# amoretti86/PSVO

Measured on AMD Instinct MI355X. Metric: particle-steps/sec, higher is better.
Workload: dtype f32

## Files before the change

### psvo_amd/csrc/bsim_bwd2_impl.h

```cpp
#pragma once
#define PSVO_BSIM_BWD_V2_UNIT 1
#include "bsim_bwd_impl.h"

namespace psvo {
PSVO_TIMERS_DEFINE(bsim_bwd2)

#define PSVO_GARG(args_type, field) ::psvo::as_global(PSVO_ARG(args_type, field))

__device__ __forceinline__ float swap_add32(float lo, float hi) {
    asm volatile("s_nop 1\n\tv_permlane32_swap_b32 %0, %1" : "+v"(lo), "+v"(hi));
    return lo + hi;
}
__device__ __forceinline__ float swap_add16(float lo, float hi) {
    asm volatile("s_nop 1\n\tv_permlane16_swap_b32 %0, %1" : "+v"(lo), "+v"(hi));
    return lo + hi;
}
__device__ __forceinline__ float row_sum16(float v) {
    v += dpp_mov<0x128, 0xF, 0xF, true>(v, v);
    v += dpp_mov<0x124, 0xF, 0xF, true>(v, v);
    v += dpp_mov<0x122, 0xF, 0xF, true>(v, v);
    v += dpp_mov<0x121, 0xF, 0xF, true>(v, v);
    return v;
}

__device__ __forceinline__ float rs_bit3(float lo, float hi) {
    float r;
    asm volatile("s_nop 1\n\t"
                 "v_add_f32_dpp %0, %1, %1 row_ror:8 row_mask:0xf bank_mask:0x3\n\t"
                 "v_add_f32_dpp %0, %2, %2 row_ror:8 row_mask:0xf bank_mask:0xc"
                 : "=&v"(r) : "v"(lo), "v"(hi));
    return r;
}
__device__ __forceinline__ float rs_bit2(float lo, float hi) {
    float r;
    asm volatile("s_nop 1\n\t"
                 "v_add_f32_dpp %0, %1, %1 row_shl:4 row_mask:0xf bank_mask:0x5\n\t"
                 "v_add_f32_dpp %0, %2, %2 row_shr:4 row_mask:0xf bank_mask:0xa"
                 : "=&v"(r) : "v"(lo), "v"(hi));
    return r;
}
template <int K>
__device__ __forceinline__ void row_reduce_scatter(const float (&v)[4 * K], float (&out)[K]) {
    float h[2 * K];
#pragma unroll
    for (int i = 0; i < 2 * K; ++i) h[i] = rs_bit3(v[i], v[2 * K + i]);
#pragma unroll
    for (int i = 0; i < K; ++i) out[i] = group_sum<4>(rs_bit2(h[i], h[K + i]));
}

typedef float f4v __attribute__((ext_vector_type(4)));
typedef __bf16 bf8v __attribute__((ext_vector_type(8)));

__device__ __forceinline__ void bf16_split3(float v, unsigned& h, unsigned& m, unsigned& l) {
    const unsigned hb = __float_as_uint(v) & 0xffff0000u;
    const float r = v - __uint_as_float(hb);
    const unsigned mb = __float_as_uint(r) & 0xffff0000u;
    const float r2 = r - __uint_as_float(mb);
    h = hb >> 16;
    m = mb >> 16;
    l = __float_as_uint(r2) >> 16;
}
__device__ __forceinline__ uint4 bf16x3_a(float v) {
    unsigned h, m, l;
    bf16_split3(v, h, m, l);
    return make_uint4(h | (h << 16), m | (h << 16), l | (m << 16), m | (l << 16));
}
__device__ __forceinline__ uint4 bf16x3_b(float v) {
    unsigned h, m, l;
    bf16_split3(v, h, m, l);
    return make_uint4(h | (m << 16), h | (l << 16), h | (m << 16), l | (m << 16));
}

template <int DX, int DY, int H, int M, int JM>
__global__ void __launch_bounds__(256, 2) bsim_bwd2_kernel(const BsimBwdArgs a) {
    using MQ = MlpLds<DX, H, DX, 1>;
    using MG = MlpLds<DX, H, DY, 1>;
    using AC = BAcc<DX>;
    constexpr int kN = AC::kSg + DY;
    constexpr int PS = (JM == 3) ? 20 : (DX == 4 && JM == 0) ? 5 : BTileSlot<DX>::kFloats;
    constexpr int FO = (JM == 3) ? 16 : 0;
    constexpr int NA = DX + 1;
    constexpr int PART = 2;
    constexpr int G = M * PART;
    constexpr int CPW = 64 / G;
    constexpr int CM = CPW * M;
    constexpr int NF = DX + 2;
    constexpr int UVS = (2 * DX + 3) & ~3;
    constexpr int JC = (JM == 0 && DX == 4) ? 2 : (JM || DX >= 3) ? 4 : 8;
    constexpr bool RO = (DX == 4) && (JM == 0);
    constexpr bool kSplitTile = (DX == 4) && (JM == 0);
    static_assert(CM == 32 && (M % 4) == 0, "two lanes per (chain, m): M in {4, 8, 16, 32}");
    extern __shared__ __attribute__((aligned(16))) float smem[];

    const int tid = threadIdx.x, lane = tid & 63, wave = tid >> 6;
    constexpr int NTB = 256, nwv = 4;
    const int B = a.B, T = a.T, N = a.N;
    const int NP = ((N + 127) / 128) * 128;
    const int nch = NP / (16 * JC);
    const int b = blockIdx.y, blk = blockIdx.x, nblk = gridDim.x;
    constexpr int cpb = nwv * CPW;
    const int cl = lane / G, part = (lane / M) & 1, m = lane % M;
    const bool h0 = (part == 0);
    const int n_raw = blk * cpb + wave * CPW + cl;
    const bool valid = n_raw < N;
    const int n = valid ? n_raw : N - 1;
    const bool srow = valid && h0;
    const bool lead = srow && (m == 0);
    const int j16 = lane & 15, g = lane >> 4;

    float* wf = smem;
    float* wg = wf + MQ::kSize;
    float* wqi = wg + MG::kSize;
    float* tile = wqi + MQ::kSize;
    float* jacc = tile + 2 * NP * PS;
    float* xch = jacc + nwv * NA * NP;
    float* uvx = xch + nwv * NF * CM;
    float* red = uvx + nwv * CM * UVS;
    float* const xw = xch + wave * NF * CM;
    float* const uw = uvx + wave * CM * UVS;
    float* const ja = jacc + wave * NA * NP;

    MQ::load(wf, a.f, tid, NTB);
    MG::load(wg, a.g, tid, NTB);
    MQ::load(wqi, a.q1inv, tid, NTB);

    const float kappa = sqrtf(0.5f * kLog2e);
    float isf[DX], rp[DX], isfk[DX], isg[DY];
#pragma unroll
    for (int d = 0; d < DX; ++d) {
        isf[d] = 1.f / a.sig_f[d];
        rp[d] = isf[d] * kappa;
        isfk[d] = isf[d] / kappa;
    }
    float ikap2 = 1.f / (kappa * kappa);
#pragma unroll
    for (int e = 0; e < DY; ++e) isg[e] = 1.f / a.sig_g[e];
    float pc[DX], pic[DX], pi1[DX], pi2[DX];
#pragma unroll
    for (int d = 0; d < DX; ++d) {
        pi1[d] = 1.f / a.sig_q1inv[d];
        pi2[d] = 1.f / a.sig_bq2[d];
        pic[d] = pi1[d] + pi2[d];
        pc[d] = 1.f / pic[d];
    }
    float s_init[DX], is_init[DX], i_isig[DX], im[DX], mi[DX];
#pragma unroll
    for (int d = 0; d < DX; ++d) {
        s_init[d] = a.sig_init[d];
        is_init[d] = 1.f / s_init[d];
        i_isig[d] = 1.f / a.isig[d];
        im[d] = a.imean[b * DX + d];
        mi[d] = a.minit[b * DX + d];
    }
    if constexpr (DX <= 2) {
        keep_in_vgpr(isf); keep_in_vgpr(rp); keep_in_vgpr(isfk); keep_in_vgpr(isg); keep_in_vgpr(ikap2);
        keep_in_vgpr(pc); keep_in_vgpr(pic); keep_in_vgpr(pi1); keep_in_vgpr(pi2);
    }
    const float ninf = -__builtin_huge_valf();
    const float aw = valid ? as_global(a.dscore)[(size_t)b * N + n] : 0.f;

    const unsigned NM = (unsigned)N * M;
    unsigned o_nm = 4u * ((unsigned)b * NM + n * M + m);
    unsigned o_dnm[DX], o_knm[DY], o_dn[DX];
#pragma unroll
    for (int d = 0; d < DX; ++d) {
        o_dnm[d] = 4u * (((unsigned)b * DX + d) * NM + n * M + m);
        o_dn[d] = 4u * (((unsigned)b * DX + d) * N + n);
    }
#pragma unroll
    for (int k = 0; k < DY; ++k) o_knm[k] = 4u * (((unsigned)b * DY + k) * NM + n * M + m);
    unsigned o_n = 4u * ((unsigned)b * N + n);
    unsigned o_d = 4u * ((unsigned)b * DX), o_k = 4u * ((unsigned)b * DY);
    const unsigned s_nm = 4u * B * NM, s_dnm = s_nm * DX, s_knm = s_nm * DY, s_dn = 4u * B * DX * N, s_n = 4u * B * N,
                   s_d = 4u * B * DX, s_k = 4u * B * DY;

    float st[DX + 1], st_l = 0.f;
    int st_t = 0;
    auto put_slot = [&](float* buf, int j, const float (&raw)[DX + 1], float l) {
        float F[DX];
#pragma unroll
        for (int d = 0; d < DX; ++d) F[d] = raw[d] * rp[d];
        const float W = j < N ? (raw[DX] - l) * kLog2e : ninf;
        if constexpr (JM == 3) {
            const float Wf = fmaxf(W, -1e30f);
            uint4* q = reinterpret_cast<uint4*>(buf + j * PS);
            q[0] = bf16x3_b(F[0]);
            q[1] = bf16x3_b(F[DX > 1 ? 1 : 0]);
            q[2] = bf16x3_b(Wf - (F[0] * F[0] + F[DX > 1 ? 1 : 0] * F[DX > 1 ? 1 : 0]));
            q[3] = bf16x3_b(1.f);
            *reinterpret_cast<float4*>(buf + j * PS + 16) = make_float4(F[0], F[DX > 1 ? 1 : 0], 0.f, 0.f);
        } else if constexpr (JM == 2) {
            *reinterpret_cast<float4*>(buf + j * PS) = make_float4(F[0], F[1], W - (F[0] * F[0] + F[DX > 1 ? 1 : 0] * F[DX > 1 ? 1 : 0]), 1.f);
        } else if constexpr (DX <= 3) {
            float4 v;
            v.x = F[0];
            v.y = DX > 1 ? F[DX > 1 ? 1 : 0] : 0.f;
            v.z = DX > 2 ? F[DX > 2 ? 2 : 0] : 0.f;
            v.w = W;
            *reinterpret_cast<float4*>(buf + j * PS) = v;
        } else if constexpr (kSplitTile) {
            *reinterpret_cast<float4*>(buf + 4 * j) = make_float4(F[0], F[1], F[2], F[3]);
            buf[4 * NP + j] = W;
        } else {
            *reinterpret_cast<float4*>(buf + j * PS) = make_float4(F[0], F[1], F[2], F[3]);
            *reinterpret_cast<float4*>(buf + j * PS + 4) = make_float4(W, 0.f, 0.f, 0.f);
        }
    };
    auto tile_entry = [&](const float* buf, int j, float (&F)[DX], float& W) {
        if constexpr (kSplitTile) {
            const float4 e = *reinterpret_cast<const float4*>(buf + 4 * j);
            F[0] = e.x; F[DX > 1 ? 1 : 0] = e.y; F[DX > 2 ? 2 : 0] = e.z; F[DX > 3 ? 3 : 0] = e.w;
            W = buf[4 * NP + j];
        } else {
            read_slot<DX>(buf + j * PS, F, W);
        }
    };
    static_assert(offsetof(BsimBwdArgs, logW) - offsetof(BsimBwdArgs, Fm) == 8 &&
                  offsetof(BsimBwdArgs, lse) - offsetof(BsimBwdArgs, Fm) == 16 && offsetof(BsimBwdArgs, Fm) % 32 == 0,
                  "BsimBwdArgs: forward-tile pointer block");
    auto get_slot = [&](int tt, int j, float (&raw)[DX + 1], gptr<const float> Fm, gptr<const float> logW) {
        const unsigned tb = (unsigned)tt * B + b;
        const unsigned jc = j < N ? j : N - 1;
#pragma unroll
        for (int d = 0; d < DX; ++d) raw[d] = ldf(Fm, 4u * ((tb * DX + d) * N + jc));
        raw[DX] = ldf(logW, 4u * (tb * N + jc));
    };
    float st2[DX + 1];
    const bool two_slots = (DX >= 3) && NP > NTB;
    auto stage_load = [&](int tt) {
        unsigned long long pt[4];
        arg_block<4>((unsigned)offsetof(BsimBwdArgs, Fm), pt);
        st_t = tt;
        const gptr<const float> p_Fm = as_global<const float>(pt[0]), p_logW = as_global<const float>(pt[1]);
        st_l = ldf(as_global<const float>(pt[2]), 4u * ((unsigned)tt * B + b));
        if (tid < NP) get_slot(tt, tid, st, p_Fm, p_logW);
        if (two_slots && tid + NTB < NP) get_slot(tt, tid + NTB, st2, p_Fm, p_logW);
    };
    auto stage_store = [&](float* buf) {
        if (tid < NP) put_slot(buf, tid, st, st_l);
        if (two_slots && tid + NTB < NP) put_slot(buf, tid + NTB, st2, st_l);
        for (int j = tid + (two_slots ? 2 : 1) * NTB; j < NP; j += NTB) {
            float raw[DX + 1];
            get_slot(st_t, j, raw, PSVO_GARG(BsimBwdArgs, Fm), PSVO_GARG(BsimBwdArgs, logW));
            put_slot(buf, j, raw, st_l);
        }
    };
    if (T >= 2) {
        stage_load(0);
        stage_store(tile);
    }
    __syncthreads();

    constexpr bool kAccLds = (DX >= 3);
    constexpr int kRowsA = 2 * DX + DY, kRowsB = 5 * DX, kSlotsB = 8;
    float acc[kAccLds ? 1 : kN];
    float* const accA = red + 16 + wave * (kRowsA * 32 + kRowsB * kSlotsB);
    float* const accB = accA + kRowsA * 32;
    auto acc_is_lead = [](int k) { return k < 4 * DX || (k >= 5 * DX && k < 6 * DX); };
    auto acc_row = [](int k) {
        return k < 4 * DX ? k : k < 5 * DX ? k - 4 * DX : k < 6 * DX ? 4 * DX + (k - 5 * DX)
               : k < 7 * DX ? DX + (k - 6 * DX) : 2 * DX + (k - 7 * DX);
    };
    const int s32 = cl * M + m;
    if constexpr (kAccLds) {
        for (int i = lane; i < kRowsA * 32 + kRowsB * kSlotsB; i += 64) accA[i] = 0.f;
    } else {
#pragma unroll
        for (int i = 0; i < kN; ++i) acc[i] = 0.f;
    }
    auto acc_add = [&](int k, float v) {
        if constexpr (kAccLds) {
            if (acc_is_lead(k)) atomicAdd(&accB[acc_row(k) * kSlotsB + cl], v);
            else atomicAdd(&accA[acc_row(k) * 32 + s32], v);
        } else {
            acc[k] += v;
        }
    };
    float dX[DX];
#pragma unroll
    for (int d = 0; d < DX; ++d) dX[d] = 0.f;

    struct StepIn {
        float eps[DX], bm[DX], xp[DX], mu1[DX], y[DY], om, lam2;
        int sel;
    };
    static_assert(offsetof(BsimBwdArgs, dscore) - offsetof(BsimBwdArgs, obs) == 56 && offsetof(BsimBwdArgs, obs) % 64 == 0 &&
                  offsetof(BsimBwdArgs, eps_b) - offsetof(BsimBwdArgs, obs) == 8 &&
                  offsetof(BsimBwdArgs, bwX) - offsetof(BsimBwdArgs, obs) == 16 &&
                  offsetof(BsimBwdArgs, sel) - offsetof(BsimBwdArgs, obs) == 24 &&
                  offsetof(BsimBwdArgs, lam2_all) - offsetof(BsimBwdArgs, obs) == 32 &&
                  offsetof(BsimBwdArgs, om_all) - offsetof(BsimBwdArgs, obs) == 40 &&
                  offsetof(BsimBwdArgs, mu1_all) - offsetof(BsimBwdArgs, obs) == 48, "BsimBwdArgs: input pointer block");
    auto load_step = [&](bool lst, bool fst, StepIn& s) {
        unsigned long long pb[8];
        arg_block<8>((unsigned)offsetof(BsimBwdArgs, obs), pb);
        const gptr<const float> p_obs = as_global<const float>(pb[0]);
        const gptr<const float> p_eps = as_global<const float>(pb[1]);
        const gptr<const float> p_bwX = as_global<const float>(pb[2]);
        const gptr<const int32_t> p_sel = as_global<const int32_t>(pb[3]);
        const gptr<const float> p_lam2 = as_global<const float>(pb[4]);
        const gptr<const float> p_om = as_global<const float>(pb[5]);
        const gptr<const float> p_mu1 = as_global<const float>(pb[6]);
        const gptr<const float> p_bm = PSVO_GARG(BsimBwdArgs, bmu2);
        s.sel = ldi(p_sel, o_n);
#pragma unroll
        for (int d = 0; d < DX; ++d) {
            s.eps[d] = ldf(p_eps, o_dnm[d]);
            s.bm[d] = ldf(p_bm, o_d + 4u * d);
            s.xp[d] = lst ? 0.f : ldf(p_bwX, o_dn[d] + s_dn);
            s.mu1[d] = lst ? 0.f : ldf(p_mu1, o_dn[d]);
        }
#pragma unroll
        for (int k = 0; k < DY; ++k) s.y[k] = ldf(p_obs, o_k + 4u * k);
        s.om = ldf(p_om, o_nm);
        s.lam2 = fst ? 0.f : ldf(p_lam2, o_nm);
    };
    auto advance = [&]() {
        o_nm += s_nm; o_n += s_n; o_d += s_d; o_k += s_k;
#pragma unroll
        for (int d = 0; d < DX; ++d) { o_dnm[d] += s_dnm; o_dn[d] += s_dn; }
#pragma unroll
        for (int k = 0; k < DY; ++k) o_knm[k] += s_knm;
    };
    auto settle = [&](StepIn& s) {
        keep_in_vgpr(s.eps); keep_in_vgpr(s.bm); keep_in_vgpr(s.xp); keep_in_vgpr(s.mu1); keep_in_vgpr(s.y);
        keep_in_vgpr(s.om); keep_in_vgpr(s.lam2);
        asm volatile("" : "+v"(s.sel));
    };
    StepIn cur_in;
    load_step(T == 1, true, cur_in);
    settle(cur_in);

    phase_skew(a.skew);
    SEC_INIT(bsim_bwd2)
    for (int t = 0; t < T; ++t) {
        SEC(0);
        const bool first = (t == 0), last = (t == T - 1);
        const float* cur = tile + ((t + 1) & 1) * NP * PS;
        float* nxt = tile + (t & 1) * NP * PS;
        constexpr bool kLateTile = (DX == 4);
        if (!kLateTile && t + 1 < T && t >= 1) stage_load(t);
        advance();
        constexpr bool kLatePrefetch = (DX >= 3);
        StepIn nxt_in;
        auto prefetch = [&]() {
            if (t + 1 < T) load_step(t + 2 == T, false, nxt_in);
            else nxt_in = StepIn{};
        };
        if (!kLatePrefetch) prefetch();
        SEC(1);

        float xp[DX], eps[DX], bm[DX], mu1[DX], mu[DX], x[DX], y[DY];
        const int sel = cur_in.sel;
#pragma unroll
        for (int d = 0; d < DX; ++d) {
            eps[d] = cur_in.eps[d];
            bm[d] = cur_in.bm[d];
            xp[d] = cur_in.xp[d];
            mu1[d] = cur_in.mu1[d];
            if (!last) {
                mu[d] = pc[d] * fmaf(pi1[d], mu1[d], pi2[d] * bm[d]);
                x[d] = fmaf(pc[d], eps[d], mu[d]);
            } else {
                mu[d] = mi[d];
                x[d] = fmaf(s_init[d], eps[d], mu[d]);
            }
        }
#pragma unroll
        for (int k = 0; k < DY; ++k) y[k] = cur_in.y[k];
        const float pi_m = valid ? exp2_fast(cur_in.om * kLog2e) : 0.f;
        const float issel = (m == sel) ? 1.f : 0.f;
        const float dphi = aw * pi_m;
        const float dlam = -aw * (issel - pi_m);

        float dxt[DX];
#pragma unroll
        for (int d = 0; d < DX; ++d) dxt[d] = h0 ? issel * dX[d] : 0.f;

        SEC(2);
        if (!first) {
            if (h0) {
#pragma unroll
                for (int d = 0; d < DX; ++d) xw[d * CM + cl * M + m] = x[d] * rp[d];
                xw[DX * CM + cl * M + m] = cur_in.lam2;
                xw[(DX + 1) * CM + cl * M + m] = dlam;
            }
            __builtin_amdgcn_fence(__ATOMIC_RELEASE, "wavefront");
            __builtin_amdgcn_wave_barrier();
            __builtin_amdgcn_fence(__ATOMIC_ACQUIRE, "wavefront");

            if constexpr (RO) {
#pragma unroll 1
                for (int r = 0; r < 2; ++r) {
                    const int it4 = 4 * (4 * r + g);
                    f2 xa[DX], xb[DX], Ua[DX], Ub[DX], Va[DX], Vb[DX];
#pragma unroll
                    for (int d = 0; d < DX; ++d) {
                        const float4 v = *reinterpret_cast<const float4*>(xw + d * CM + it4);
                        xa[d] = f2{v.x, v.y};
                        xb[d] = f2{v.z, v.w};
                        Ua[d] = Ub[d] = Va[d] = Vb[d] = f2{0.f, 0.f};
                    }
                    const float4 lq = *reinterpret_cast<const float4*>(xw + DX * CM + it4);
                    const float4 dl = *reinterpret_cast<const float4*>(xw + (DX + 1) * CM + it4);
                    const f2 lqa = f2{lq.x, lq.y}, lqb = f2{lq.z, lq.w};
                    const f2 dla = f2{dl.x, dl.y}, dlb = f2{dl.z, dl.w};
#pragma unroll 1
                    for (int c = 0; c < nch; ++c) {
                        float A2[JC][NA];
#pragma unroll
                        for (int jt = 0; jt < JC; ++jt) {
                            float F[DX], W;
                            tile_entry(cur, (c * JC + jt) * 16 + j16, F, W);
                            f2 ua[DX], ub[DX], la = f2{W, W}, lb = la;
#pragma unroll
                            for (int d = 0; d < DX; ++d) {
                                const f2 Fd = f2{F[d], F[d]};
                                ua[d] = xa[d] - Fd;
                                ub[d] = xb[d] - Fd;
                                la = pk_fma(-ua[d], ua[d], la);
                                lb = pk_fma(-ub[d], ub[d], lb);
                            }
// ... 208 lines not shown
                    if (g == 0 || DX > 3) {
#pragma unroll
                        for (int jt = 0; jt < JC; ++jt) {
                            float F[DX], W;
                            read_slot<DX>(cbase + jt * 16 * PS, F, W);
                            (void)W;
                            const int j = (c * JC + jt) * 16 + j16;
                            if constexpr (DX <= 3) {
                                const float sc = D4[jt][DX];
#pragma unroll
                                for (int d = 0; d < DX; ++d) ja[d * NP + j] = D4[jt][d] - F[d] * sc;
                                ja[DX * NP + j] = sc;
                            } else {
                                const float sc = __shfl(D4[jt][0], 16 + j16);
                                if (g == 0) {
#pragma unroll
                                    for (int d = 0; d < DX; ++d) ja[d * NP + j] = D4[jt][d] - F[d] * sc;
                                    ja[DX * NP + j] = sc;
                                }
                            }
                        }
                    }
                }
            }
#pragma unroll
            for (int r = 0; r < 2; ++r) {
                float vv[4 * 2 * DX], o[UVS];
#pragma unroll
                for (int d = 0; d < DX; ++d) {
                    vv[0 * 2 * DX + d] = Ua[r][d].x; vv[1 * 2 * DX + d] = Ua[r][d].y;
                    vv[2 * 2 * DX + d] = Ub[r][d].x; vv[3 * 2 * DX + d] = Ub[r][d].y;
                    vv[0 * 2 * DX + DX + d] = Va[r][d].x; vv[1 * 2 * DX + DX + d] = Va[r][d].y;
                    vv[2 * 2 * DX + DX + d] = Vb[r][d].x; vv[3 * 2 * DX + DX + d] = Vb[r][d].y;
                }
                float red2[2 * DX];
                row_reduce_scatter<2 * DX>(vv, red2);
#pragma unroll
                for (int e = 0; e < UVS; ++e) o[e] = e < 2 * DX ? red2[e < 2 * DX ? e : 0] : 0.f;
                if ((j16 & 3) == 0) {
                    float* dst = uw + (4 * (4 * r + g) + (j16 >> 2)) * UVS;
#pragma unroll
                    for (int e = 0; e < UVS; e += 4)
                        *reinterpret_cast<float4*>(dst + e) = make_float4(o[e], o[e + 1], o[e + 2], o[e + 3]);
                }
            }
            }
            __builtin_amdgcn_fence(__ATOMIC_RELEASE, "wavefront");
            __builtin_amdgcn_wave_barrier();
            __builtin_amdgcn_fence(__ATOMIC_ACQUIRE, "wavefront");
            SEC(3);
            if (h0) {
                float uv[UVS];
#pragma unroll
                for (int e = 0; e < UVS; e += 4) {
                    const float4 q4 = *reinterpret_cast<const float4*>(uw + (cl * M + m) * UVS + e);
                    uv[e] = q4.x; uv[e + 1] = q4.y; uv[e + 2] = q4.z; uv[e + 3] = q4.w;
                }
                if constexpr (JM >= 2) {
#pragma unroll
                    for (int d = 0; d < DX; ++d) {
                        const float xs = x[d] * rp[d], r1 = uv[d], r2 = uv[DX + d];
                        uv[d] = xs - r1;
                        uv[DX + d] = fmaf(xs, xs - 2.f * r1, r2);
                    }
                }
#pragma unroll
                for (int d = 0; d < DX; ++d) {
                    dxt[d] -= dlam * uv[d] * isfk[d];
                    acc_add(AC::kSf + d, dlam * (uv[DX + d] * ikap2 - 1.f) * isf[d]);
                }
            }
        } else {
#pragma unroll
            for (int d = 0; d < DX; ++d) {
                const float z = (x[d] - im[d]) * i_isig[d];
                const float tz = dphi * z * i_isig[d];
                if (h0) {
                    dxt[d] -= tz;
                    acc_add(AC::kSiota + d, dphi * (z * z - 1.f) * i_isig[d]);
                }
            }
        }

        if (kLatePrefetch) prefetch();
        if (kLateTile && t + 1 < T && t >= 1) stage_load(t);
        SEC(4);
        float dxp_part[DX];
#pragma unroll
        for (int d = 0; d < DX; ++d) dxp_part[d] = 0.f;
        {
            float dFo[DX];
#pragma unroll
            for (int d = 0; d < DX; ++d) dFo[d] = 0.f;
            if (!last) {
                float fmx[DX];
                MQ::template eval_part<PART>(wf, part, x, fmx);
#pragma unroll
                for (int d = 0; d < DX; ++d) fmx[d] += xor_lane<M>(fmx[d]);
#pragma unroll
                for (int d = 0; d < DX; ++d) {
                    const float z = (xp[d] - fmx[d]) * isf[d];
                    dFo[d] = dphi * z * isf[d];
                    if (h0) {
                        dxp_part[d] = -dFo[d];
                        acc_add(AC::kSf + d, dphi * (z * z - 1.f) * isf[d]);
                    }
                }
                MQ::template bwd_input_part<PART>(wf, part, x, dFo, dxt);
            }
            static_assert(offsetof(BsimBwdArgs, dFt) - offsetof(BsimBwdArgs, xt) == 8 &&
                          offsetof(BsimBwdArgs, dGt) - offsetof(BsimBwdArgs, xt) == 16 &&
                          offsetof(BsimBwdArgs, dmu1) - offsetof(BsimBwdArgs, xt) == 24 && offsetof(BsimBwdArgs, xt) % 32 == 0,
                          "BsimBwdArgs: row pointer block");
            unsigned long long pr[4];
            arg_block<4>((unsigned)offsetof(BsimBwdArgs, xt), pr);
            if (srow) {
#pragma unroll
                for (int d = 0; d < DX; ++d) {
                    stf(as_global<float>(pr[1]), o_dnm[d] - s_dnm, dFo[d]);
                    stf(as_global<float>(pr[0]), o_dnm[d] - s_dnm, x[d]);
                }
            }
            float gm[DY], dGo[DY];
            MG::template eval_part<PART>(wg, part, x, gm);
#pragma unroll
            for (int k = 0; k < DY; ++k) gm[k] += xor_lane<M>(gm[k]);
#pragma unroll
            for (int k = 0; k < DY; ++k) {
                float dmean = 1.f;
                if (a.emission) { dmean = emis_dmean(gm[k]); gm[k] = emis_mean(gm[k]); }
                const float z = (y[k] - gm[k]) * isg[k];
                dGo[k] = dphi * z * isg[k] * dmean;
                if (h0) acc_add(AC::kSg + k, dphi * (z * z - 1.f) * isg[k]);
                if (srow) stf(as_global<float>(pr[2]), o_knm[k] - s_knm, dGo[k]);
            }
            MG::template bwd_input_part<PART>(wg, part, x, dGo, dxt);
        }

        SEC(5);
        float dmu[DX], sce[DX], dxp[DX], dim[DX];
#pragma unroll
        for (int d = 0; d < DX; ++d) {
            const float v3 = (first && h0) ? dphi * (x[d] - im[d]) * i_isig[d] * i_isig[d] : 0.f;
            dmu[d] = group_sum<G>(dxt[d]);
            sce[d] = group_sum<G>(dxt[d] * eps[d]);
            dxp[d] = group_sum<G>(dxp_part[d]);
            dim[d] = first ? group_sum<G>(v3) : 0.f;
        }
        float outv[DX];
        if (!last) {
            float dmu1[DX];
#pragma unroll
            for (int d = 0; d < DX; ++d) {
                dmu1[d] = dmu[d] * pc[d] * pi1[d];
                outv[d] = dmu[d] * pc[d] * pi2[d];
                if (lead) {
                    stf(PSVO_GARG(BsimBwdArgs, dmu1), o_dn[d] - s_dn, dmu1[d]);
                    acc_add(AC::kSc + d, sce[d] + aw * pic[d]);
                    acc_add(AC::kSmm1 + d, dmu[d] * mu1[d]);
                    acc_add(AC::kSmb + d, dmu[d] * bm[d]);
                    acc_add(AC::kSmm + d, dmu[d] * mu[d]);
                }
            }
            {
                constexpr int kQS = (H / 4 < G) ? H / 4 : G;
                float dq[DX];
#pragma unroll
                for (int d = 0; d < DX; ++d) dq[d] = 0.f;
                MQ::template bwd_input_part<kQS>(wqi, (lane % G) & (kQS - 1), xp, dmu1, dq);
#pragma unroll
                for (int d = 0; d < DX; ++d) dxp[d] += group_sum<kQS>(dq[d]);
            }
        } else {
#pragma unroll
            for (int d = 0; d < DX; ++d) {
                outv[d] = dmu[d];
                if (lead) {
                    stf(PSVO_GARG(BsimBwdArgs, dmu1), o_dn[d] - s_dn, 0.f);
                    acc_add(AC::kSinit + d, sce[d] + aw * is_init[d]);
                }
            }
        }
#pragma unroll
        for (int d = 0; d < DX; ++d) dX[d] = dxp[d];
        if (lead) {
#pragma unroll
            for (int d = 0; d < DX; ++d) {
                stf(PSVO_GARG(BsimBwdArgs, dbmu2_rows), o_dn[d] - s_dn, last ? 0.f : outv[d]);
                if (last) PSVO_GARG(BsimBwdArgs, dminit_rows)[((size_t)b * DX + d) * N + n] = outv[d];
                if (first) PSVO_GARG(BsimBwdArgs, dimean_rows)[((size_t)b * DX + d) * N + n] = dim[d];
            }
        }
        SEC(6);
        __syncthreads();
        settle(nxt_in);
        cur_in = nxt_in;
        const size_t tb = (size_t)t * B + b;
        if (!first) {
            const size_t tbm = tb - B;
            const gptr<float> pF = PSVO_GARG(BsimBwdArgs, dFm_part) + (tbm * nblk + blk) * DX * N;
            const gptr<float> pW = PSVO_GARG(BsimBwdArgs, dlogW_part) + (tbm * nblk + blk) * N;
            for (int j = tid; j < N; j += NTB) {
#pragma unroll
                for (int d = 0; d < NA; ++d) {
                    const float* col = jacc + d * NP + j;
                    const float a0 = col[0], a1 = col[NA * NP], a2 = col[2 * NA * NP], a3 = col[3 * NA * NP];
                    const float s = (a0 + a1) + (a2 + a3);
                    if (d < DX) pF[d * N + j] = s * isfk[d < DX ? d : 0];
                    else pW[j] = s;
                }
            }
        }
        if (last) {
            const gptr<float> pF = PSVO_GARG(BsimBwdArgs, dFm_part) + (tb * nblk + blk) * DX * N;
            const gptr<float> pW = PSVO_GARG(BsimBwdArgs, dlogW_part) + (tb * nblk + blk) * N;
            for (int j = tid; j < N; j += NTB) {
#pragma unroll
                for (int d = 0; d < DX; ++d) pF[d * N + j] = 0.f;
                pW[j] = 0.f;
            }
        }
        SEC(7);
        if (t + 1 < T && t >= 1) stage_store(nxt);
        __syncthreads();
        SEC(8);
    }

    for (int i = 0; i < kN; ++i) {
        float v = 0.f;
        if constexpr (kAccLds) {
            if (acc_is_lead(i)) v = lane < kSlotsB ? accB[acc_row(i) * kSlotsB + lane] : 0.f;
            else v = lane < 32 ? accA[acc_row(i) * 32 + lane] : 0.f;
        } else {
#pragma unroll
            for (int k = 0; k < kN; ++k) v = (k == i) ? acc[k] : v;
        }
        v = wave_sum(v);
        if (lane == 0) red[wave] = v;
        __syncthreads();
        if (tid == 0) {
            float s = 0.f;
            for (int w = 0; w < nwv; ++w) s += red[w];
            as_global(a.sacc_part)[((size_t)b * nblk + blk) * kN + i] = s;
        }
        __syncthreads();
    }
}

static inline void bsim2_geometry(int N, int M, int& cpb, int& nblk) {
    cpb = 4 * (64 / (2 * M));
    nblk = (N + cpb - 1) / cpb;
}

static inline bool bsim2_supported(int B, int T, int N, int M, int Dx, int Dy) {
    if (pick_m(M, [](auto) { return PSVO_OK; }) != PSVO_OK) return false;
    const long long big = (long long)T * B * (Dx > Dy ? Dx : Dy) * N * M * 4;
    return big < (1ll << 32);
}

template <int DX, int DY, int H, int M>
static int launch_bsim_bwd2(const BsimBwdArgs& a, const BsimBwdOut& o, int jm, hipStream_t stream) {
    using MQ = MlpLds<DX, H, DX, 1>;
    using MG = MlpLds<DX, H, DY, 1>;
    const int PS = (jm == 3 && DX == 2) ? 20 : (DX == 4) ? 5 : BTileSlot<DX>::kFloats;
    constexpr int UVS = (2 * DX + 3) & ~3;
    int cpb, nblk;
    bsim2_geometry(a.N, M, cpb, nblk);
    const int NP = ((a.N + 127) / 128) * 128;
    const size_t lds = sizeof(float) * (2 * MQ::kSize + MG::kSize + 2 * (size_t)NP * PS + 4 * (size_t)(DX + 1) * NP +
                                        4 * (DX + 2) * 32 + 4 * 32 * UVS + 16 +
                                        (DX >= 3 ? 4 * ((2 * DX + DY) * 32 + 5 * DX * 8) : 0));
    if (lds > 160 * 1024) return PSVO_ERR_UNSUPPORTED;
    BsimBwdArgs as = a;
    as.skew = (int)(2560.0 * NP / 128.0 * (3 * DX + 4) / 10.0 * g_tune_skew_pct / 100.0);
    clear_hip_error();
    if (jm == 3 && DX == 2) {
        if constexpr (DX == 2)
            hipLaunchKernelGGL((bsim_bwd2_kernel<DX, DY, H, M, 3>), dim3(nblk, a.B), dim3(256), lds, stream, as);
    } else if (jm == 2 && DX == 2) {
        if constexpr (DX == 2)
            hipLaunchKernelGGL((bsim_bwd2_kernel<DX, DY, H, M, 2>), dim3(nblk, a.B), dim3(256), lds, stream, as);
    } else if (jm == 1 && DX == 2) {
        if constexpr (DX == 2)
            hipLaunchKernelGGL((bsim_bwd2_kernel<DX, DY, H, M, 1>), dim3(nblk, a.B), dim3(256), lds, stream, as);
    } else {
        hipLaunchKernelGGL((bsim_bwd2_kernel<DX, DY, H, M, 0>), dim3(nblk, a.B), dim3(256), lds, stream, as);
    }
    (void)o;
    return launch_status();
}

template <int DX>
int bb2_dispatch_dy(const BsimBwdArgs& a, const BsimBwdOut& o, int Dy, int H, int M, int jm, hipStream_t s) {
    return dispatch_dy_h_m(Dy, H, M, [&](auto dy, auto h, auto m) __attribute__((visibility("hidden"))) {
        return launch_bsim_bwd2<DX, dy(), h(), m()>(a, o, jm, s); });
}

}
```

### psvo_amd/csrc/filter_fwd.hip

```cpp
#include "common.h"

namespace psvo {
inline namespace PSVO_LNS {
PSVO_TIMERS_DEFINE(filter_fwd)


struct FilterArgs {
    int B, T, N;
    int resample, two_q, bootstrap, emission;
    psvo_mlp q1, f, g;
    const float *sig_q1, *sig_q2, *sig_f, *sig_g;
    const float *mu2, *m0, *sig0, *fm0, *fsig0, *obs, *eps, *u;
    const int32_t* idx_in;
    float *X, *Xanc, *Fm, *P1, *logW;
    int32_t* idx_out;
    float* lse;
};

template <int DX, int DY, int H, int MAXT, int EM = 2>
__global__ void __launch_bounds__(MAXT) filter_fwd_kernel(const FilterArgs a) {
    using MQ = MlpLds<DX, H, DX, PSVO_L>;
    using MG = MlpLds<DX, H, DY, PSVO_L>;
    extern __shared__ __attribute__((aligned(16))) float smem[];

// ... 144 lines not shown
        } else {
            total = lane_bcast(sc, 63);
        }
        const float lse_t = fmaf(kLn2, log2_fast(total), mx);
        if (tid == 0) a.lse[tb] = lse_t;

        SEC(5);
        if (a.resample) {
            cdf[tid] = sc;
#pragma unroll
            for (int d = 0; d < DX; ++d) {
                sx[d * NT + tid] = x[d];
                sp[d * NT + tid] = p1[d];
                if (!a.bootstrap) sf[d * NT + tid] = fm[d];
            }
            __syncthreads();
            SEC(6);
            int idx;
            if (a.idx_in) {
                idx = idx_c;
            } else {
                const float target = u_c * total;
                int pos = 0;
                for (int s = 1 << (31 - __clz(N)); s > 0; s >>= 1) {
                    const int p = pos + s;
                    if (p <= N && cdf[p - 1] <= target) pos = p;
                }
                idx = min(pos, N - 1);
            }
#pragma unroll
            for (int d = 0; d < DX; ++d) {
                x[d] = sx[d * NT + idx];
                mean1[d] = sp[d * NT + idx];
                fmean[d] = a.bootstrap ? mean1[d] : sf[d * NT + idx];
            }
            if (valid) {
                a.idx_out[tb * N + n] = idx;
#pragma unroll
                for (int d = 0; d < DX; ++d) a.Xanc[(tb * DX + d) * N + n] = x[d];
            }
            lnw = neg_logN;
            SEC(7);
            __syncthreads();
        } else {
#pragma unroll
            for (int d = 0; d < DX; ++d) {
                mean1[d] = p1[d];
                fmean[d] = fm[d];
            }
            if (valid) {
                a.idx_out[tb * N + n] = n;
#pragma unroll
                for (int d = 0; d < DX; ++d) a.Xanc[(tb * DX + d) * N + n] = x[d];
            }
            lnw = lw - lse_t;
            if (nw > 1) __syncthreads();
        }

#pragma unroll
        for (int d = 0; d < DX; ++d) {
            eps_c[d] = eps_n[d];
            mu2_c[d] = mu2_n[d];
        }
#pragma unroll
        for (int k = 0; k < DY; ++k) obs_c[k] = obs_n[k];
        u_c = u_n;
        idx_c = idx_n;
    }
}

template <int DX, int DY, int H, int MAXT>
__global__ void __launch_bounds__(MAXT) filter_fwd_lpp_kernel(const FilterArgs a) {
    using MQ = MlpLds<DX, H, DX, PSVO_L>;
    using MG = MlpLds<DX, H, DY, PSVO_L>;
    constexpr int P = 4;
    constexpr bool kOpaque = false;
    extern __shared__ __attribute__((aligned(16))) float smem[];

    const int tid = threadIdx.x, lane = tid & 63, wave = tid >> 6;
    const int NT = blockDim.x, nw = NT >> 6;
    const int NPT = NT / P;
    const int b = blockIdx.x, B = a.B, T = a.T, N = a.N;
    const int pn = tid >> 2, p = tid & 3;
    const int uwave = __builtin_amdgcn_readfirstlane(wave);
    const bool valid = pn < N;
    const int n = valid ? pn : N - 1;

    float* wq1 = smem;
    float* wf = wq1 + MQ::kSize;
    float* wg = wf + MQ::kSize;
    float* cdf = wg + MG::kSize;
    float* piv = cdf + NPT;
    float* sx = piv + 16;
    float* sp = sx + DX * NPT;
    float* sf = sp + DX * NPT;
    float* red = sf + DX * NPT;

    MQ::load(wq1, a.q1, tid, NT);
    if (!a.bootstrap) MQ::load(wf, a.f, tid, NT);
    MG::load(wg, a.g, tid, NT);
    const float* wfm = a.bootstrap ? wq1 : wf;
    if (tid < 16) piv[tid] = __builtin_huge_valf();

    float sq1[DX], sq2[DX], sfv[DX], s0[DX], fs0[DX], isg[DY];
    float lg = -DY * kHalfLog2Pi;
#pragma unroll
    for (int d = 0; d < DX; ++d) {
        sq1[d] = a.sig_q1[d];
        sq2[d] = a.two_q ? a.sig_q2[d] : 1.f;
        sfv[d] = a.bootstrap ? a.sig_q1[d] : a.sig_f[d];
        s0[d] = a.sig0[d];
        fs0[d] = a.fsig0[d];
    }
#pragma unroll
    for (int e = 0; e < DY; ++e) {
        const float s = a.sig_g[e];
        isg[e] = 1.f / s;
        lg -= logf(s);
    }
    const StepK<DX> K0 = make_stepk<DX>(s0, sq2, fs0, a.two_q != 0);
    const StepK<DX> K1 = make_stepk<DX>(sq1, sq2, sfv, a.two_q != 0);
    const float neg_logN = -logf((float)N);
    const float ninf = -__builtin_huge_valf();

    float mean1[DX], fmean[DX];
#pragma unroll
    for (int d = 0; d < DX; ++d) {
        mean1[d] = a.m0[b * DX + d];
        fmean[d] = a.fm0[b * DX + d];
    }
    float lnw = neg_logN;

    constexpr int kFU = DX, kFM2 = DX + 1, kFY = 2 * DX + 1, kFields = 2 * DX + 1 + DY, kSlots = (kFields + 3) / 4;
    const in_word_t* in_ptr[kSlots];
    int in_str[kSlots];
    auto field_ptr = [&](int f, const in_word_t*& q, int& st) {
        q = a.eps + (size_t)b * DX * N + n;
        st = 0;
        if (f < kFU) {
            q = a.eps + ((size_t)b * DX + f) * N + n;
            st = B * DX * N;
        } else if (f == kFU) {
            if (a.resample) {
                q = (a.idx_in ? reinterpret_cast<const in_word_t*>(a.idx_in) : static_cast<const in_word_t*>(a.u)) + (size_t)b * N + n;
                st = B * N;
            }
        } else if (f < kFY) {
            if (a.two_q) {
                q = a.mu2 + (size_t)b * DX + (f - kFM2);
                st = B * DX;
            }
        } else if (f < kFields) {
            q = a.obs + (size_t)b * DY + (f - kFY);
            st = B * DY;
        }
    };
#pragma unroll
    for (int s = 0; s < kSlots; ++s) {
        field_ptr(4 * s, in_ptr[s], in_str[s]);
#pragma unroll
        for (int j = 1; j < 4; ++j) {
            const in_word_t* q;
            int st;
            field_ptr(4 * s + j, q, st);
            in_ptr[s] = (p == j) ? q : in_ptr[s];
            in_str[s] = (p == j) ? st : in_str[s];
        }
    }
    float eps_c[DX], mu2_c[DX], obs_c[DY], u_c = 0.f;
    int idx_c = 0;
    float raw_n[kSlots];
    auto issue_inputs = [&]() {
#pragma unroll
        for (int s = 0; s < kSlots; ++s) {
            raw_n[s] = *in_ptr[s];
            in_ptr[s] += in_str[s];
        }
    };
    auto take_inputs = [&]() {
#pragma unroll
        for (int d = 0; d < DX; ++d) {
            eps_c[d] = quad_field(raw_n, d);
            const float m = quad_field(raw_n, kFM2 + d);
            mu2_c[d] = a.two_q ? m : 0.f;
        }
#pragma unroll
        for (int k = 0; k < DY; ++k) obs_c[k] = quad_field(raw_n, kFY + k);
        u_c = quad_field(raw_n, kFU);
        idx_c = __builtin_bit_cast(int, u_c);
    };
    issue_inputs();
    take_inputs();
    __syncthreads();

    SEC_INIT(filter_fwd)
    auto step = [&](auto first_tag, const int t) {
        SEC(0);
        const size_t tb = (size_t)t * B + b;
        const StepK<DX> K = decltype(first_tag)::value ? K0 : K1;
        if (t + 1 < T) issue_inputs();

        SEC(1);
        float mu[DX], x[DX];
#pragma unroll
        for (int d = 0; d < DX; ++d) {
            mu[d] = a.two_q ? K.c[d] * fmaf(K.i1[d], mean1[d], K.i2[d] * mu2_c[d]) : mean1[d];
            x[d] = fmaf(K.c[d], eps_c[d], mu[d]);
        }
        const float q_lp = diag_lp<DX>(x, mu, K.ic, K.lq);
        const float f_lp = diag_lp<DX>(x, fmean, K.ifs, K.lf);

        SEC(2);
        int zo = 0;
        if (kOpaque) asm volatile("" : "+v"(zo));
        float gm[DY], p1[DX], fm[DX];
        MG::template eval_part<P>(wg + zo, p, x, gm);
        MQ::template eval_part<P>(wq1 + zo, p, x, p1);
        if (!a.bootstrap) MQ::template eval_part<P>(wfm + zo, p, x, fm);
#pragma unroll
        for (int k = 0; k < DY; ++k) gm[k] = group_sum<P>(gm[k]);
        if (a.emission) {
#pragma unroll
            for (int k = 0; k < DY; ++k) gm[k] = emis_mean(gm[k]);
        }
#pragma unroll
        for (int d = 0; d < DX; ++d) {
            p1[d] = group_sum<P>(p1[d]);
            fm[d] = a.bootstrap ? p1[d] : group_sum<P>(fm[d]);
        }
        const float g_lp = diag_lp<DY>(obs_c, gm, isg, lg);
        float lw = f_lp + g_lp - q_lp + lnw;
        if (!valid) lw = ninf;

        if (valid) {
            if (p == 0) {
#pragma unroll
                for (int d = 0; d < DX; ++d) a.X[(tb * DX + d) * N + n] = x[d];
                a.logW[tb * N + n] = lw;
            } else if (p == 1) {
#pragma unroll
                for (int d = 0; d < DX; ++d) a.Fm[(tb * DX + d) * N + n] = fm[d];
            } else if (p == 2 && a.P1) {
#pragma unroll
                for (int d = 0; d < DX; ++d) a.P1[(tb * DX + d) * N + n] = p1[d];
            }
        }

        SEC(3);
        const float wmx = wave_max(lw);
        const float wbase = (wmx == ninf) ? 0.f : wmx;
        const float w = (valid && p == 0) ? exp2_fast((lw - wbase) * kLog2e) : 0.f;
        float sc = wave_incl_scan(w, lane);
        if (lane == 63) {
            red[wave] = wmx;
            red[16 + wave] = sc;
        }
        if (a.resample) {
            if (p == 1) {
#pragma unroll
                for (int d = 0; d < DX; ++d) sx[d * NPT + pn] = x[d];
            } else if (p == 2) {
#pragma unroll
                for (int d = 0; d < DX; ++d) sp[d * NPT + pn] = p1[d];
            } else if (p == 3 && !a.bootstrap) {
#pragma unroll
                for (int d = 0; d < DX; ++d) sf[d * NPT + pn] = fm[d];
            }
        }
        SEC(4);
        __syncthreads();
        SEC(5);
        const int li = lane & 15;
        const float m_i = li < nw ? red[li] : ninf;
        const float s_i = li < nw ? red[16 + li] : 0.f;
        const float gmx = lane_bcast(group_max<16>(m_i), 0);
        const float gbase = (gmx == ninf) ? 0.f : gmx;
        const float v_i = s_i * exp2_fast((m_i - gbase) * kLog2e);
        const float pre = group_incl_scan<16>(v_i, li);
        const float total = lane_bcast(pre, nw - 1);
        const float off = uwave > 0 ? lane_bcast(pre, max(uwave - 1, 0)) : 0.f;
        sc = fmaf(sc, exp2_fast((wbase - gbase) * kLog2e), off);
        const float lse_t = fmaf(kLn2, log2_fast(total), gmx);
        if (tid == 3) a.lse[tb] = lse_t;

        SEC(6);
        if (a.resample) {
            if (p == 0) {
                cdf[pn] = sc;
                if ((pn & 15) == 15) piv[pn >> 4] = sc;
            }
            __syncthreads();
            SEC(7);
            int idx;
            if (a.idx_in) {
                idx = idx_c;
            } else {
                const float target = u_c * total;
                const float4 pv = *reinterpret_cast<const float4*>(piv + 4 * p);
                float c1 = (pv.x <= target ? 1.f : 0.f) + (pv.y <= target ? 1.f : 0.f) +
                           (pv.z <= target ? 1.f : 0.f) + (pv.w <= target ? 1.f : 0.f);
                c1 = group_sum<P>(c1);
                const int blk = min((int)c1, (NPT >> 4) - 1);
                const float4 cv = *reinterpret_cast<const float4*>(cdf + 16 * blk + 4 * p);
                float c2 = (cv.x <= target ? 1.f : 0.f) + (cv.y <= target ? 1.f : 0.f) +
                           (cv.z <= target ? 1.f : 0.f) + (cv.w <= target ? 1.f : 0.f);
                c2 = group_sum<P>(c2);
                idx = min(16 * blk + (int)c2, N - 1);
            }
#pragma unroll
            for (int d = 0; d < DX; ++d) {
                x[d] = sx[d * NPT + idx];
                mean1[d] = sp[d * NPT + idx];
                fmean[d] = a.bootstrap ? mean1[d] : sf[d * NPT + idx];
            }
            if (valid) {
                if (p == 3) a.idx_out[tb * N + n] = idx;
                if (p == 0) {
#pragma unroll
                    for (int d = 0; d < DX; ++d) a.Xanc[(tb * DX + d) * N + n] = x[d];
                }
            }
            lnw = neg_logN;
            SEC(8);
            __syncthreads();
            SEC(9);
        } else {
#pragma unroll
            for (int d = 0; d < DX; ++d) {
                mean1[d] = p1[d];
                fmean[d] = fm[d];
            }
            if (valid) {
                if (p == 3) a.idx_out[tb * N + n] = n;
                if (p == 0) {
#pragma unroll
                    for (int d = 0; d < DX; ++d) a.Xanc[(tb * DX + d) * N + n] = x[d];
                }
            }
            lnw = lw - lse_t;
            __syncthreads();
        }

        take_inputs();
    };
    step(std::true_type{}, 0);
    for (int t = 1; t < T; ++t) step(std::false_type{}, t);
}

template <int DX, int DY, int H>
static int launch_filter(const FilterArgs& a, hipStream_t stream) {
    using MQ = MlpLds<DX, H, DX, PSVO_L>;
    using MG = MlpLds<DX, H, DY, PSVO_L>;
    constexpr bool kLppOk = (H % 16 == 0) && (PSVO_L == 2 || (H <= 32 && DX <= 3) || H == 16);
    if constexpr (kLppOk) {
        if (a.N <= 128) {
            const int NT4 = (4 * a.N + 63) & ~63;
            const int NPT = NT4 / 4;
            const size_t lds4 = sizeof(float) * (2 * MQ::kSize + MG::kSize + NPT + 16 + 3 * DX * NPT + 32);
            clear_hip_error();
            hipLaunchKernelGGL((filter_fwd_lpp_kernel<DX, DY, H, 512>), dim3(a.B), dim3(NT4), lds4, stream, a);
            return launch_status();
        }
    }
    const int NT = (a.N + 63) & ~63;
    const size_t lds = sizeof(float) * (2 * MQ::kSize + MG::kSize + NT + 3 * DX * NT + 48);
    clear_hip_error();
    if (NT <= 256 && a.emission)
        hipLaunchKernelGGL((filter_fwd_kernel<DX, DY, H, 256, 1>), dim3(a.B), dim3(NT), lds, stream, a);
    else if (NT <= 256)
        hipLaunchKernelGGL((filter_fwd_kernel<DX, DY, H, 256, 0>), dim3(a.B), dim3(NT), lds, stream, a);
    else
        hipLaunchKernelGGL((filter_fwd_kernel<DX, DY, H, 512>), dim3(a.B), dim3(NT), lds, stream, a);
    return launch_status();
}

}
}

PSVO_L2_DECL(psvo_filter_forward)
PSVO_ENTRY(psvo_filter_forward)(const psvo_desc* desc, const psvo_mlp* q1, const psvo_mlp* f, const psvo_mlp* g,
                                   const float* sig_q1, const float* sig_q2, const float* sig_f,
                                   const float* sig_g, const float* mu2, const float* m0, const float* sig0,
                                   const float* fm0, const float* fsig0, const float* obs, const float* eps,
                                   const float* u, const int32_t* idx_in, float* X, float* Xanc, float* Fm, float* P1,
                                   float* logW, int32_t* idx_out, float* lse, void* stream) {
    using namespace psvo;
    if (!desc_layers_ok(desc) || !desc_emission_ok(desc)) return PSVO_ERR_UNSUPPORTED;
#if PSVO_L == 1
    if (desc && desc->layers == 2)
        return psvo_filter_forward_l2(desc, q1, f, g, sig_q1, sig_q2, sig_f, sig_g, mu2, m0, sig0, fm0, fsig0, obs,
            eps, u, idx_in, X, Xanc, Fm, P1, logW, idx_out, lse, stream);
#endif
    if (!mlp_layers_ok(q1) || !mlp_layers_ok(f) || !mlp_layers_ok(g)) return PSVO_ERR_INVALID;
    if (!desc || !q1 || !g || !sig_q1 || !sig_g || !m0 || !sig0 || !fm0 || !fsig0 || !obs || !eps || !X ||
        !Xanc || !Fm || !logW || !idx_out || !lse)
        return PSVO_ERR_INVALID;
    if (desc->B <= 0 || desc->T <= 0 || desc->N <= 0) return PSVO_ERR_INVALID;
    if (desc->two_q && (!mu2 || !sig_q2)) return PSVO_ERR_INVALID;
    if (!desc->bootstrap && (!f || !sig_f)) return PSVO_ERR_INVALID;
    if (desc->resample && !u && !idx_in) return PSVO_ERR_INVALID;
    if (desc->N > 512) return PSVO_ERR_UNSUPPORTED;

    FilterArgs a;
    a.B = desc->B; a.T = desc->T; a.N = desc->N;
    a.resample = desc->resample; a.two_q = desc->two_q; a.bootstrap = desc->bootstrap; a.emission = desc->emission;
    a.q1 = *q1; a.f = desc->bootstrap ? *q1 : *f; a.g = *g;
    a.sig_q1 = sig_q1; a.sig_q2 = sig_q2; a.sig_f = sig_f; a.sig_g = sig_g;
    a.mu2 = mu2; a.m0 = m0; a.sig0 = sig0; a.fm0 = fm0; a.fsig0 = fsig0;
    a.obs = obs; a.eps = eps; a.u = u; a.idx_in = idx_in;
    a.X = X; a.Xanc = Xanc; a.Fm = Fm; a.P1 = P1; a.logW = logW; a.idx_out = idx_out; a.lse = lse;
    hipStream_t s = static_cast<hipStream_t>(stream);
    return dispatch_shape(desc->Dx, desc->Dy, desc->H, [&](auto dx, auto dy, auto h) {
        return launch_filter<dx(), dy(), h()>(a, s); });
}
```

Before: 258.6 million.

## Double-buffer LDS staging to drop per-step barriers in bwd and filter kernels

In the backward simulation kernel, the Jacobian accumulator is double-buffered when LDS allows (DX<=3), so the tile stage-store moves before the existing barrier and the second per-step barrier is removed. In the lpp filter kernel, the per-step staging area (cdf, particle state, reductions) is double-buffered by timestep parity. The resampling pivot search now computes block pivots from the scan partial sums in registers instead of writing rescaled CDF and pivots to LDS, which removes two barriers per step. The cost is more LDS, which can lower occupancy, plus more register work to rescale CDF entries during the search.

```diff
diff --git a/psvo_amd/csrc/bsim_bwd2_impl.h b/psvo_amd/csrc/bsim_bwd2_impl.h
--- a/psvo_amd/csrc/bsim_bwd2_impl.h
+++ b/psvo_amd/csrc/bsim_bwd2_impl.h
@@ -69,6 +69,17 @@
     unsigned h, m, l;
     bf16_split3(v, h, m, l);
     return make_uint4(h | (m << 16), h | (l << 16), h | (m << 16), l | (m << 16));
+}
+
+template <int DX, int DY, int H>
+__host__ __device__ constexpr int bsim2_lds_floats(int NP, int PS, int njb) {
+    constexpr int UVS = (2 * DX + 3) & ~3;
+    return 2 * MlpLds<DX, H, DX, 1>::kSize + MlpLds<DX, H, DY, 1>::kSize + 2 * NP * PS + njb * 4 * (DX + 1) * NP +
+           4 * (DX + 2) * 32 + 4 * 32 * UVS + 16 + (DX >= 3 ? 4 * ((2 * DX + DY) * 32 + 5 * DX * 8) : 0);
+}
+template <int DX, int DY, int H>
+__host__ __device__ constexpr int bsim2_jacc_copies(int NP, int PS) {
+    return (DX <= 3 && 4 * bsim2_lds_floats<DX, DY, H>(NP, PS, 2) <= 80 * 1024) ? 2 : 1;
 }
 
 template <int DX, int DY, int H, int M, int JM>
@@ -89,6 +100,7 @@
     constexpr int JC = (JM == 0 && DX == 4) ? 2 : (JM || DX >= 3) ? 4 : 8;
     constexpr bool RO = (DX == 4) && (JM == 0);
     constexpr bool kSplitTile = (DX == 4) && (JM == 0);
+    constexpr bool kOneBarrier = (DX <= 3);
     static_assert(CM == 32 && (M % 4) == 0, "two lanes per (chain, m): M in {4, 8, 16, 32}");
     extern __shared__ __attribute__((aligned(16))) float smem[];
 
@@ -112,13 +124,14 @@
     float* wg = wf + MQ::kSize;
     float* wqi = wg + MG::kSize;
     float* tile = wqi + MQ::kSize;
+    const int njb = kOneBarrier ? bsim2_jacc_copies<DX, DY, H>(NP, PS) : 1;
+    const bool one_barrier = kOneBarrier && njb == 2;
     float* jacc = tile + 2 * NP * PS;
-    float* xch = jacc + nwv * NA * NP;
+    float* xch = jacc + njb * nwv * NA * NP;
     float* uvx = xch + nwv * NF * CM;
     float* red = uvx + nwv * CM * UVS;
     float* const xw = xch + wave * NF * CM;
     float* const uw = uvx + wave * CM * UVS;
-    float* const ja = jacc + wave * NA * NP;
 
     MQ::load(wf, a.f, tid, NTB);
     MG::load(wg, a.g, tid, NTB);
@@ -174,7 +187,7 @@
     const unsigned s_nm = 4u * B * NM, s_dnm = s_nm * DX, s_knm = s_nm * DY, s_dn = 4u * B * DX * N, s_n = 4u * B * N,
                    s_d = 4u * B * DX, s_k = 4u * B * DY;
 
-    float st[DX + 1], st_l = 0.f;
+    float st[DX + 1] = {}, st_l = 0.f;
     int st_t = 0;
     auto put_slot = [&](float* buf, int j, const float (&raw)[DX + 1], float l) {
         float F[DX];
@@ -225,7 +238,7 @@
         for (int d = 0; d < DX; ++d) raw[d] = ldf(Fm, 4u * ((tb * DX + d) * N + jc));
         raw[DX] = ldf(logW, 4u * (tb * N + jc));
     };
-    float st2[DX + 1];
+    float st2[DX + 1] = {};
     const bool two_slots = (DX >= 3) && NP > NTB;
     auto stage_load = [&](int tt) {
         unsigned long long pt[4];
@@ -338,6 +351,8 @@
         const bool first = (t == 0), last = (t == T - 1);
         const float* cur = tile + ((t + 1) & 1) * NP * PS;
         float* nxt = tile + (t & 1) * NP * PS;
+        float* const jacc_t = jacc + (t & (njb - 1)) * nwv * NA * NP;
+        float* const ja = jacc_t + wave * NA * NP;
         constexpr bool kLateTile = (DX == 4);
         if (!kLateTile && t + 1 < T && t >= 1) stage_load(t);
         advance();
@@ -712,6 +727,11 @@
             }
         }
 
+        if constexpr (kOneBarrier) {
+            keep_in_vgpr(st);
+            keep_in_vgpr(st_l);
+            if constexpr (DX >= 3) keep_in_vgpr(st2);
+        }
         if (kLatePrefetch) prefetch();
         if (kLateTile && t + 1 < T && t >= 1) stage_load(t);
         SEC(4);
@@ -822,6 +842,7 @@
             }
         }
         SEC(6);
+        if (one_barrier && t + 1 < T && t >= 1) stage_store(nxt);
         __syncthreads();
         settle(nxt_in);
         cur_in = nxt_in;
@@ -833,7 +854,7 @@
             for (int j = tid; j < N; j += NTB) {
 #pragma unroll
                 for (int d = 0; d < NA; ++d) {
-                    const float* col = jacc + d * NP + j;
+                    const float* col = jacc_t + d * NP + j;
                     const float a0 = col[0], a1 = col[NA * NP], a2 = col[2 * NA * NP], a3 = col[3 * NA * NP];
                     const float s = (a0 + a1) + (a2 + a3);
                     if (d < DX) pF[d * N + j] = s * isfk[d < DX ? d : 0];
@@ -851,8 +872,10 @@
             }
         }
         SEC(7);
-        if (t + 1 < T && t >= 1) stage_store(nxt);
-        __syncthreads();
+        if (!one_barrier) {
+            if (t + 1 < T && t >= 1) stage_store(nxt);
+            __syncthreads();
+        }
         SEC(8);
     }
 
@@ -890,16 +913,11 @@
 
 template <int DX, int DY, int H, int M>
 static int launch_bsim_bwd2(const BsimBwdArgs& a, const BsimBwdOut& o, int jm, hipStream_t stream) {
-    using MQ = MlpLds<DX, H, DX, 1>;
-    using MG = MlpLds<DX, H, DY, 1>;
     const int PS = (jm == 3 && DX == 2) ? 20 : (DX == 4) ? 5 : BTileSlot<DX>::kFloats;
-    constexpr int UVS = (2 * DX + 3) & ~3;
     int cpb, nblk;
     bsim2_geometry(a.N, M, cpb, nblk);
     const int NP = ((a.N + 127) / 128) * 128;
-    const size_t lds = sizeof(float) * (2 * MQ::kSize + MG::kSize + 2 * (size_t)NP * PS + 4 * (size_t)(DX + 1) * NP +
-                                        4 * (DX + 2) * 32 + 4 * 32 * UVS + 16 +
-                                        (DX >= 3 ? 4 * ((2 * DX + DY) * 32 + 5 * DX * 8) : 0));
+    const size_t lds = sizeof(float) * (size_t)bsim2_lds_floats<DX, DY, H>(NP, PS, bsim2_jacc_copies<DX, DY, H>(NP, PS));
     if (lds > 160 * 1024) return PSVO_ERR_UNSUPPORTED;
     BsimBwdArgs as = a;
     as.skew = (int)(2560.0 * NP / 128.0 * (3 * DX + 4) / 10.0 * g_tune_skew_pct / 100.0);
diff --git a/psvo_amd/csrc/filter_fwd.hip b/psvo_amd/csrc/filter_fwd.hip
--- a/psvo_amd/csrc/filter_fwd.hip
+++ b/psvo_amd/csrc/filter_fwd.hip
@@ -250,25 +250,19 @@
     const int NPT = NT / P;
     const int b = blockIdx.x, B = a.B, T = a.T, N = a.N;
     const int pn = tid >> 2, p = tid & 3;
-    const int uwave = __builtin_amdgcn_readfirstlane(wave);
     const bool valid = pn < N;
     const int n = valid ? pn : N - 1;
 
     float* wq1 = smem;
     float* wf = wq1 + MQ::kSize;
     float* wg = wf + MQ::kSize;
-    float* cdf = wg + MG::kSize;
-    float* piv = cdf + NPT;
-    float* sx = piv + 16;
-    float* sp = sx + DX * NPT;
-    float* sf = sp + DX * NPT;
-    float* red = sf + DX * NPT;
+    const int blk_floats = (1 + 3 * DX) * NPT + 32;
+    float* const stage = wg + MG::kSize;
 
     MQ::load(wq1, a.q1, tid, NT);
     if (!a.bootstrap) MQ::load(wf, a.f, tid, NT);
     MG::load(wg, a.g, tid, NT);
     const float* wfm = a.bootstrap ? wq1 : wf;
-    if (tid < 16) piv[tid] = __builtin_huge_valf();
 
     float sq1[DX], sq2[DX], sfv[DX], s0[DX], fs0[DX], isg[DY];
     float lg = -DY * kHalfLog2Pi;
@@ -366,6 +360,11 @@
         SEC(0);
         const size_t tb = (size_t)t * B + b;
         const StepK<DX> K = decltype(first_tag)::value ? K0 : K1;
+        float* const cdf = stage + (t & 1) * blk_floats;
+        float* const sx = cdf + NPT;
+        float* const sp = sx + DX * NPT;
+        float* const sf = sp + DX * NPT;
+        float* const red = sf + DX * NPT;
         if (t + 1 < T) issue_inputs();
 
         SEC(1);
@@ -418,13 +417,15 @@
         const float wmx = wave_max(lw);
         const float wbase = (wmx == ninf) ? 0.f : wmx;
         const float w = (valid && p == 0) ? exp2_fast((lw - wbase) * kLog2e) : 0.f;
-        float sc = wave_incl_scan(w, lane);
+        const float sc = wave_incl_scan(w, lane);
         if (lane == 63) {
             red[wave] = wmx;
             red[16 + wave] = sc;
         }
         if (a.resample) {
-            if (p == 1) {
+            if (p == 0) {
+                cdf[pn] = sc;
+            } else if (p == 1) {
 #pragma unroll
                 for (int d = 0; d < DX; ++d) sx[d * NPT + pn] = x[d];
             } else if (p == 2) {
@@ -446,32 +447,28 @@
         const float v_i = s_i * exp2_fast((m_i - gbase) * kLog2e);
         const float pre = group_incl_scan<16>(v_i, li);
         const float total = lane_bcast(pre, nw - 1);
-        const float off = uwave > 0 ? lane_bcast(pre, max(uwave - 1, 0)) : 0.f;
-        sc = fmaf(sc, exp2_fast((wbase - gbase) * kLog2e), off);
         const float lse_t = fmaf(kLn2, log2_fast(total), gmx);
         if (tid == 3) a.lse[tb] = lse_t;
 
         SEC(6);
         if (a.resample) {
-            if (p == 0) {
-                cdf[pn] = sc;
-                if ((pn & 15) == 15) piv[pn >> 4] = sc;
-            }
-            __syncthreads();
-            SEC(7);
             int idx;
             if (a.idx_in) {
                 idx = idx_c;
             } else {
                 const float target = u_c * total;
-                const float4 pv = *reinterpret_cast<const float4*>(piv + 4 * p);
-                float c1 = (pv.x <= target ? 1.f : 0.f) + (pv.y <= target ? 1.f : 0.f) +
-                           (pv.z <= target ? 1.f : 0.f) + (pv.w <= target ? 1.f : 0.f);
-                c1 = group_sum<P>(c1);
-                const int blk = min((int)c1, (NPT >> 4) - 1);
+                const float base_i = (m_i == ninf) ? 0.f : m_i;
+                const float E_i = exp2_fast((base_i - gbase) * kLog2e);
+                const float off_i = dpp_mov<0x111, 0xF, 0xF, true>(0.f, pre);
+                const float piv_i = li < nw ? fmaf(s_i, E_i, off_i) : __builtin_huge_valf();
+                int c1 = 0;
+#pragma unroll
+                for (int i = 0; i < MAXT / 64; ++i) c1 += (lane_bcast(piv_i, i) <= target) ? 1 : 0;
+                const int blk = min(c1, nw - 1);
+                const float E_b = lane_fetch(E_i, blk), off_b = lane_fetch(off_i, blk);
                 const float4 cv = *reinterpret_cast<const float4*>(cdf + 16 * blk + 4 * p);
-                float c2 = (cv.x <= target ? 1.f : 0.f) + (cv.y <= target ? 1.f : 0.f) +
-                           (cv.z <= target ? 1.f : 0.f) + (cv.w <= target ? 1.f : 0.f);
+                float c2 = (fmaf(cv.x, E_b, off_b) <= target ? 1.f : 0.f) + (fmaf(cv.y, E_b, off_b) <= target ? 1.f : 0.f) +
+                           (fmaf(cv.z, E_b, off_b) <= target ? 1.f : 0.f) + (fmaf(cv.w, E_b, off_b) <= target ? 1.f : 0.f);
                 c2 = group_sum<P>(c2);
                 idx = min(16 * blk + (int)c2, N - 1);
             }
@@ -490,8 +487,6 @@
             }
             lnw = neg_logN;
             SEC(8);
-            __syncthreads();
-            SEC(9);
         } else {
 #pragma unroll
             for (int d = 0; d < DX; ++d) {
@@ -506,7 +501,6 @@
                 }
             }
             lnw = lw - lse_t;
-            __syncthreads();
         }
 
         take_inputs();
@@ -524,7 +518,7 @@
         if (a.N <= 128) {
             const int NT4 = (4 * a.N + 63) & ~63;
             const int NPT = NT4 / 4;
-            const size_t lds4 = sizeof(float) * (2 * MQ::kSize + MG::kSize + NPT + 16 + 3 * DX * NPT + 32);
+            const size_t lds4 = sizeof(float) * (2 * MQ::kSize + MG::kSize + 2 * ((1 + 3 * DX) * NPT + 32));
             clear_hip_error();
             hipLaunchKernelGGL((filter_fwd_lpp_kernel<DX, DY, H, 512>), dim3(a.B), dim3(NT4), lds4, stream, a);
             return launch_status();
```

Result: no change. 260.3 million (median of 6 runs) (+0.6%).
